# kevinh-e/BetaOne

Measured on AMD Instinct MI355X. Metric: mcts_nodes_per_sec, higher is better.
Workload: dtype f32 (3 x f16 split, f32 accumulate)

## Files before the change

### betaone_amd/csrc/bo_analyse.h

```cpp
#pragma once
#include "bo_tree.h"

#define BO_PV_CAP 16
#define BO_ANALYSIS_WORDS 32
#define ST_BAD_RANGE 128

BO_DEV bo_mv move_between(const DPos &P, const DPos &C) {
    const int us = pos_turn(P) ? BB_WHITE : BB_BLACK;
    uint64_t left = P.bb[us] & ~C.bb[us], arrived = C.bb[us] & ~P.bb[us];
    if (left & P.bb[BB_K]) { left &= P.bb[BB_K]; arrived &= C.bb[BB_K]; }
    if (!left || !arrived) return 0;
    const int from = bo_lsb64(left), to = bo_lsb64(arrived);
    int promo = 0;
    if ((P.bb[BB_P] & BIT(from)) && !(C.bb[BB_P] & BIT(to))) promo = piece_type_at(C, to);
    return MV(from, to, promo);
}

struct SetupDevArgs {
    const int *slots;
    const DPos *pos;
    long long capacity;
    const long long *first;
    const int *ply;
};
// ... 8 lines not shown
    int st = 0;
    if (ply < 0 || f < 0 || f + (long long)ply >= a.capacity) st = ST_BAD_RANGE;
    else if (ply + 1 > e.c.PLY_CAP) st = ST_PLY_OVERFLOW;
    else if (ply + 1 > e.c.TRK_CAP) st = ST_TRK_OVERFLOW;
    if (lane == 0) {
        e.status[g] = st;
        e.ctx_mode[g] = 0;
        e.stat_evals[g] = e.stat_flushes[g] = e.stat_term_sims[g] = e.stat_levels[g] = e.stat_children_scanned[g] = 0;
        e.resign_cnt[2 * g] = e.resign_cnt[2 * g + 1] = 0;
    }
    if (st) {
        if (lane == 0) {
            const size_t no = NOFF(e, g);
            e.ply[g] = 0; e.trk_n[g] = 0; e.n_hist[g] = 0;
            e.n_nodes[g] = 1; e.n_children[no] = 0; e.n_visits[no] = 0; e.q[no] = 0.0f;
            e.sims_done[g] = 0; e.rows[g] = 0; e.n_runs[g] = 0; e.n_ul[g] = 0; e.req_node[g] = -1; e.phase[g] = PH_IDLE; e.root_nch[g] = 0;
            e.root_nlegal[g] = 0; e.req_nlegal[g] = 0; e.root_term[g] = -1;
        }
        return;
    }
    DPos *gp = e.gpos + (size_t)g * e.c.PLY_CAP;
    DPos *tk = e.trk + (size_t)g * e.c.TRK_CAP;
    int *tc = e.trk_cnt + (size_t)g * e.c.TRK_CAP;
    bo_mv *pl = e.played + (size_t)g * e.c.PLY_CAP;
    for (int k0 = 0; k0 <= ply; k0 += 64) {
        const int k = k0 + lane;
        if (k <= ply) {
            DPos p = a.pos[f + k];
            if (k == 0) { p.flags |= F_IRREV; finish_key(p); }
            gp[k] = p;
            tk[k] = p;
// ... 77 lines not shown
```

### betaone_amd/csrc/bo_engine.cpp

```cpp
#include "../../include/betaone_engine.h"
#include "../../include/betaone_lab.h"

#include "bo_tree.h"
#include "bo_fastw.h"
#include "bo_select_wide.h"
#include "bo_replay.h"
#include "bo_train.h"
#include "bo_metrics.h"
#include "bo_pgn.h"
#include "bo_san.h"
#include "bo_analyse.h"
#include "bo_perft.h"
#include "bo_tb.h"
#include "bo_nn_fused.h"
#include "bo_conv.h"
#include "bo_tower.h"
#include "bo_tower_wg.h"
#include "bo_tower_h.h"
#include "bo_tower_s.h"
#include "bo_tower_s16.h"
#include "bo_tower_h16.h"
#include "bo_heads.h"
#include "bo_tower_b1.h"
#include "bo_rt.h"
// ... 205 lines not shown
    for (int k = 1; k <= cfg->mcts_batch_size; k++) {
        const double r = (double)(int)(cfg->widen_coeff * sqrt((double)k)) / (double)k;
        if (r > per_sim) per_sim = r;
    }
    c.NCAP = fast ? 2 : (int)ceil(c.S * per_sim) + 2 * root_m + 4;
    c.nstride = c.NCAP;
    c.PLY_CAP = cfg->max_plies; c.TRK_CAP = cfg->max_plies;
    c.UL_MAX = fast ? 1 : c.B; c.CH_MAX = ch_max < 1 ? 1 : ch_max;
    c.cpuct = (float)cfg->cpuct;
    c.keep = (float)(1.0 - cfg->dirichlet_epsilon);
    c.eps = cfg->dirichlet_epsilon;
    c.use_noise = cfg->dirichlet_alpha > 0 ? 1 : 0;
    c.root_m = root_m;
    c.profile = 0;
    { const char *v = getenv("BETAONE_BURST_TWO_PATHS"); c.burst_two = (v && v[0] == '0') ? 0 : 1; }
    c.root_q = 0;
    const size_t G = (size_t)c.G, N = G * (size_t)c.NCAP;
    Eng &d = e->d;
    int rc = 0;
    float *sq = nullptr, *rcp = nullptr; int *wl = nullptr;
    rc |= e->alloc(&sq, (size_t)c.S + 2); rc |= e->alloc(&wl, (size_t)c.B + 1); rc |= e->alloc(&rcp, (size_t)c.S + 3);
    int **iscal[] = {&d.sims_done, &d.n_nodes, &d.rows, &d.n_runs, &d.n_ul, &d.req_nlegal, &d.status,
                     &d.trk_n, &d.n_hist, &d.ctx_mode, &d.root_nch, &d.stat_evals,
                     &d.stat_flushes, &d.stat_term_sims, &d.stat_levels, &d.stat_children_scanned, &e->d_go, &e->d_action};
    for (int **p : iscal) rc |= e->alloc(p, G);
    const size_t res_ints = G * (4 + 2 * (size_t)BO_RES_CAP) + 4, info_ints = G * 18;
    rc |= e->alloc(&e->d_res_blk, res_ints); rc |= e->alloc(&e->d_info_blk, info_ints);
    if (!rc) {
        d.res_n = e->d_res_blk; d.res_best_idx = e->d_res_blk + G; d.res_best_mv = e->d_res_blk + 2 * G; d.res_total = e->d_res_blk + 3 * G;
        d.res_idx = e->d_res_blk + 4 * G; d.res_val = reinterpret_cast<float *>(e->d_res_blk + 4 * G + G * BO_RES_CAP);
// ... 8 lines not shown
    rc |= rt_host_alloc((void **)&e->h_res, res_ints * 4); rc |= rt_host_alloc((void **)&e->h_info, info_ints * 4);
    rc |= rt_host_alloc((void **)&e->h_noise, G * BO_MAX_MOVES * sizeof(double)); rc |= rt_host_alloc((void **)&e->h_go, G * 4);
    rc |= rt_host_alloc((void **)&e->h_action, 2 * G * 4);
    rc |= rt_host_alloc((void **)&e->h_turn_u, G * sizeof(double)); rc |= rt_host_alloc((void **)&e->h_turn_flags, G * 4);
    rc |= e->alloc(&e->d_turn_pw, (size_t)cfg->num_simulations + 1);
    { const char *v = getenv("BETAONE_TURN_COPIES"); e->ship = !(v && v[0] == '1'); }
    rc |= e->alloc(&d.gpos, G * c.PLY_CAP); rc |= e->alloc(&d.trk, G * c.TRK_CAP); rc |= e->alloc(&d.trk_cnt, G * c.TRK_CAP);
    rc |= e->alloc(&d.hist, G * 7);
    rc |= e->alloc(&d.n_visits, N); rc |= e->alloc(&d.parent, N); rc |= e->alloc(&d.first_child, N); rc |= e->alloc(&d.n_children, N);
    rc |= e->alloc(&d.q, N); rc |= e->alloc(&d.prior, N); rc |= e->alloc(&d.move, N); rc |= e->alloc(&d.term, N);
    rc |= e->alloc(&d.eval_slot, N); rc |= e->alloc(&d.npos, N);
    rc |= e->alloc(&d.run_leaf, G * c.B); rc |= e->alloc(&d.run_cnt, G * c.B);
    rc |= e->alloc(&d.ul_node, G * c.UL_MAX); rc |= e->alloc(&d.ul_nlegal, G * c.UL_MAX); rc |= e->alloc(&d.ul_value, G * c.UL_MAX);
    rc |= e->alloc(&d.ul_move, G * c.UL_MAX * BO_CH_CAP); rc |= e->alloc(&d.ul_prior, G * c.UL_MAX * BO_CH_CAP);
    rc |= e->alloc(&d.req_moves, G * BO_MAX_MOVES); rc |= e->alloc(&d.root_moves, G * BO_MAX_MOVES);
    rc |= e->alloc(&d.root_child_rank, G * 2 * BO_CH_CAP); rc |= e->alloc(&d.noise, G * BO_MAX_MOVES);
    rc |= e->alloc(&d.played, G * c.PLY_CAP);
    rc |= e->alloc(&d.prof, G * BO_PROF_SLOTS);
    rc |= e->alloc(&d.resign_cnt, 2 * G); rc |= e->alloc(&e->d_root_value, G);
    if (!rc) rt_memset(d.resign_cnt, 0, 2 * G * 4, nullptr);
    d.played_now = nullptr;
    if (fast) {
        FastW &f = e->f;
        const size_t L = (size_t)cfg->leaves_per_step;
        f.L = (int)L;
        f.sel_ut = 2; f.sel_flags = FW_SEL_OCT;
        const size_t expansions = (size_t)c.S + L + 2;
        f.NG = cfg->fast_arena_granules > 0 ? cfg->fast_arena_granules : (int)((6 * expansions + 8) * (32 / BO_FW_GR));
        if (f.NG < 64 || f.NG > BO_FW_LINK_MASK) { bo_engine_destroy(e); return fail(BO_E_ARG, "fast_arena_granules out of range (64 .. 2^24 - 1)"); }
        const size_t NR = (size_t)f.NG * BO_FW_GR;
// ... 251 lines not shown
            if (e->sel_pending) {
                float ms = 0.0f;
                RT((int)hipEventSynchronize(e->sel_ev1));
                RT((int)hipEventElapsedTime(&ms, e->sel_ev0, e->sel_ev1));
                e->sel_ms += ms; e->sel_launches++; e->sel_pending = 0;
            }
            RT((int)hipEventRecord(e->sel_ev0, (hipStream_t)stream));
        }
#endif
        RT(launch_fw_select(e, value_dev, policy_kind, stream));
#if !defined(BO_WAVE_EMU)
        if (e->sel_profile) { RT((int)hipEventRecord(e->sel_ev1, (hipStream_t)stream)); e->sel_pending = 1; }
#endif
        RT(RT_LAUNCH(bo_k_fw_leaf, rows, stream, e->d, e->f, nn_in_dev));
    } else {
        RT(RT_LAUNCH(bo_k_step, e->d.c.G, stream, e->d, policy_dev, value_dev, policy_kind, nn_in_dev, vt));
    }
    return BO_OK;
}
extern "C" int bo_step(bo_engine *e, const float *policy_dev, const float *value_dev, int policy_kind, float *nn_in_dev,
                       void *stream) {
    if (!e || !nn_in_dev) return fail(BO_E_ARG, "null argument");
    if (policy_kind != BO_POLICY_NONE && (!policy_dev || !value_dev)) return fail(BO_E_ARG, "policy/value required");
    return step_launch(e, policy_dev, value_dev, policy_kind, nn_in_dev, stream, StepTail{nullptr, nullptr, nullptr, nullptr, 0});
}
extern "C" int bo_step_heads(bo_engine *e, const float *logits_dev, const float *vpart_dev, const float *b1_dev, const float *w2_dev,
                             const float *b2_dev, int rows, float *nn_in_dev, void *stream) {
    if (!e || !nn_in_dev || !logits_dev || !vpart_dev || !b1_dev || !w2_dev || !b2_dev) return fail(BO_E_ARG, "null argument");
    if (e->fast) return fail(BO_E_CONFIG, "bo_step_heads: the reference-semantics search only (fast mode evaluates rows, not games)");
    if (rows < e->d.c.G) return fail(BO_E_ARG, "bo_step_heads: the partial sums must hold a row per game (rows >= G)");
    return step_launch(e, logits_dev, nullptr, BO_POLICY_LOGITS, nn_in_dev, stream, StepTail{vpart_dev, b1_dev, w2_dev, b2_dev, rows});
// ... 1257 lines not shown
    RT(rt_sync(stream));
    return BO_OK;
}

extern "C" int bo_debug_profile(bo_engine *e, int enable, uint64_t *cycles_out, void *stream) {
    if (!e) return fail(BO_E_ARG, "null engine");
    const size_t G = (size_t)e->d.c.G;
    if (cycles_out) {
        RT(rt_d2h(cycles_out, e->d.prof, G * BO_PROF_SLOTS * sizeof(uint64_t), stream));
        RT(rt_sync(stream));
    }
    if (enable >= 0) {
        if (enable && !e->d.c.profile) RT(rt_memset(e->d.prof, 0, G * BO_PROF_SLOTS * sizeof(uint64_t), stream));
        e->d.c.profile = enable;
    }
    return BO_OK;
}

extern "C" int bo_movegen_batch(bo_engine *e, int n, const bo_position *pos, int32_t *moves_out, int32_t *n_out,
                                int32_t *check_out, void *stream) {
    if (!e || n < 1 || !pos || !moves_out || !n_out) return fail(BO_E_ARG, "bad arguments");
    std::vector<DPos> hp((size_t)n);
    for (int i = 0; i < n; i++) hp[i] = from_abi(pos[i]);
    void *dp = nullptr, *dm = nullptr, *dn = nullptr, *dc = nullptr;
    int rc = rt_malloc(&dp, hp.size() * sizeof(DPos)) | rt_malloc(&dm, (size_t)n * BO_MAX_MOVES * sizeof(bo_mv)) |
             rt_malloc(&dn, (size_t)n * 4) | rt_malloc(&dc, (size_t)n * 4);
    std::vector<bo_mv> hm((size_t)n * BO_MAX_MOVES);
    std::vector<int> hc((size_t)n);
    if (!rc) rc = rt_h2d(dp, hp.data(), hp.size() * sizeof(DPos), stream);
    if (!rc) rc = RT_LAUNCH(bo_k_movegen, n, stream, (const DPos *)dp, (bo_mv *)dm, (int *)dn, (int *)dc);
// ... 1192 lines not shown
```

### betaone_amd/csrc/bo_tree.h

```cpp
#pragma once
#include "bo_chess.h"
#include <math.h>

#define BO_CH_CAP 32
#define BO_PATH_CAP 1024
#define BO_RES_CAP 256
#define BO_PLANES 120
#ifndef BO_PROF_SLOTS
#define BO_PROF_SLOTS 16
#endif
#define BO_ROW (BO_PLANES * 64)

enum { PH_IDLE = 0, PH_RUN = 1, PH_DONE = 2 };
enum { ST_OK = 0, ST_NODE_OVERFLOW = 1, ST_DEPTH_OVERFLOW = 2, ST_NAN_SCORE = 4, ST_PLY_OVERFLOW = 8,
       ST_ILLEGAL_ACTION = 16, ST_UL_OVERFLOW = 32, ST_TRK_OVERFLOW = 64 };
enum { POLICY_NONE = 0, POLICY_LOGITS = 1, POLICY_PROBS = 2 };

struct EngCfg {
    int G, S, B;
    int NCAP, PLY_CAP, TRK_CAP;
    int nstride;
    int UL_MAX, CH_MAX;
    float cpuct, keep;
    double eps;
    int use_noise;
    int root_m;
    int profile;
    int burst_two;
    int root_q;
};

struct Eng {
    EngCfg c;
    const float *sqrt_lut;
    const float *rcp_lut;
    const int *widen_lut;
    int *phase, *sims_done, *n_nodes, *rows, *n_runs, *n_ul, *req_node, *req_nlegal, *status;
    int *ply, *trk_n, *n_hist, *ctx_mode, *root_nlegal, *root_term, *root_nch;
    int *stat_evals, *stat_flushes, *stat_term_sims, *stat_levels, *stat_children_scanned;
    DPos *gpos, *trk, *hist;
    int *trk_cnt;
    int *n_visits, *parent, *first_child, *n_children;
    float *q, *prior;
    bo_mv *move;
    signed char *term;
    short *eval_slot;
    DPos *npos;
    int *run_leaf, *run_cnt;
    int *ul_node, *ul_nlegal;
    float *ul_value;
    bo_mv *ul_move;
    float *ul_prior;
    bo_mv *req_moves, *root_moves;
    int *root_child_rank;
    double *noise;
    bo_mv *played;
    int *res_n, *res_idx, *res_best_idx, *res_best_mv, *res_total;
    float *res_val;
    int watch_n;
    int *watch, *res_watch;
    int *played_now;
    int *resign_cnt;
    unsigned long long *prof;
};

#define NOFF(e, g) ((size_t)(g) * (size_t)(e).c.nstride)

BO_DEV float bo_expf(float x) {
// ... 196 lines not shown
BO_DEV void encode_static(const Eng &e, int g, float *row) {
    const int s = bo_lane();
    const int nh = e.n_hist[g];
    const DPos *h = e.hist + (size_t)g * 7;
    for (int pl = 0; pl < (7 - nh) * 14; pl++) row[pl * 64 + s] = 0.0f;
    for (int i = 0; i < nh; i++) {
        DPos H = h[i];
        encode_block(row, 7 - nh + i, H, tracker_reps(e, g, H));
    }
}
BO_DEV void encode_leaf(const Eng &e, int g, float *row, const DPos &P) {
    encode_block(row, 7, P, tracker_reps(e, g, P));
    encode_scalars(row, P);
}

BO_DEV int select_leaf(const Eng &e, int g, int *flags, int *path, int *depth_out, const float *lut) {
    const size_t no = NOFF(e, g);
    const int lane = bo_lane();
    int cur = 0, levels = 0, scanned = 0;
    if (lane == 0) path[0] = 0;
    int nc = e.n_children[no], fc = e.first_child[no];
    int pv = e.n_visits[no], pv_next = pv;
    for (;;) {
        if (nc == 0) break;
        const float sp = lut[pv];
        float score = -__builtin_inff();
        int n = 0, c_fc = 0, c_nc = 0;
        if (lane < nc) {
            n = e.n_visits[no + fc + lane];
            c_fc = e.first_child[no + fc + lane];
            c_nc = e.n_children[no + fc + lane];
// ... 28 lines not shown
        score = __builtin_bit_cast(float, bo_readlane(__builtin_bit_cast(int, score), 0));
        bi = bo_readlane(bi, 0);
        if (!(score > -__builtin_inff())) { *flags |= ST_NAN_SCORE; bi = 0; }
        cur = fc + bi;
        levels++;
        if (lane == 0) path[levels] = cur;
        scanned += nc;
        pv = pv_next;
        pv_next = bo_readlane(n, bi);
        fc = bo_readlane(c_fc, bi);
        nc = bo_readlane(c_nc, bi);
        if (levels >= BO_PATH_CAP - 1) { *flags |= ST_DEPTH_OVERFLOW; break; }
    }
    if (lane == 0) { e.stat_levels[g] += levels; e.stat_children_scanned[g] += scanned; }
    *depth_out = levels;
    bo_sync();
    return cur;
}

#define BO_BURST_LEVELS 4
#define BO_BURST_FITS(S) (2 * (S) + 5 <= BO_NUM_ACTIONS)
BO_DEV_NOINLINE float bo_div_general(float x, float fn) { return x / fn; }
BO_DEV float bo_div_count(float x, float fn, float y) {
    const float q0 = x * y;
    const float r = __builtin_fmaf(-fn, q0, x);
    float q = __builtin_fmaf(r, y, q0);
    const float a = q0 < 0.0f ? -q0 : q0;
    if (x == 0.0f) q = q0;
    else if (!(a >= 1e-30f && a <= 1e30f)) q = bo_div_general(x, fn);
    return q;
// ... 391 lines not shown
    BO_UNROLL
    for (int w = 0; w < 4; w++) {
        float h = 0.0f;
        BO_UNROLL
        for (int ks = 0; ks < 16; ks++) h += r.part[w][ks];
        h += r.b1[w];
        s[w] = (h > 0.0f ? h : 0.0f) * r.w2[w];
    }
    for (int m = 32; m >= 1; m >>= 1) {
        BO_UNROLL
        for (int w = 0; w < 4; w++) s[w] = s[w] + bo_shfl_xor_f(s[w], m);
    }
    return tanhf(((s[0] + s[1]) + (s[2] + s[3])) + r.b2);
}

BO_DEV void apply_leaf(const Eng &e, int g, int leaf, const float *row, int kind, const float *value_of, const StepTail &vt, StepShared &sh,
                       int *n_ul_io, int *flags) {
    const size_t no = NOFF(e, g);
    const int lane = bo_lane();
    const int n = e.req_nlegal[g];
    const bo_mv *mv = e.req_moves + (size_t)g * BO_MAX_MOVES;
    int slot = *n_ul_io;
    if (slot >= e.c.UL_MAX) { *flags |= ST_UL_OVERFLOW; slot = e.c.UL_MAX - 1; }
    const size_t uo = (size_t)g * e.c.UL_MAX + slot;
    float value;
    if (kind == POLICY_PROBS) {
        value = value_of[g];
        for (int j = lane; j < n; j += 64) sh.pv[j] = row[move_to_index(mv[j])];
    } else {
        float mx, sum;
        if (vt.vpart) {
            TailRegs tr;
            tail_load(vt, g, tr);
            row_max_sum(row, &mx, &sum);
            value = tail_value(tr);
        } else {
            value = value_of[g];
            row_max_sum(row, &mx, &sum);
        }
        for (int j = lane; j < n; j += 64) sh.pv[j] = bo_exp_row(row[move_to_index(mv[j])] - mx) / sum;
    }
    bo_sync();
    const int M = n < e.c.CH_MAX ? n : e.c.CH_MAX;
    for (int j = lane; j < n; j += 64) {
        int r = stable_rank(sh.pv, n, j);
        if (r < M) { e.ul_move[uo * BO_CH_CAP + r] = mv[j]; e.ul_prior[uo * BO_CH_CAP + r] = sh.pv[j]; }
    }
    if (lane == 0) {
        e.ul_node[uo] = leaf;
        e.ul_nlegal[uo] = n;
        e.ul_value[uo] = value;
        e.eval_slot[no + leaf] = (short)slot;
    }
    *n_ul_io = slot + 1;
    bo_sync();
}


BO_DEV int step_body(const Eng &e, int g, const float *policy, const float *value, int kind, float *nn_in, StepShared &sh, const StepTail &vt) {
    const int lane = bo_lane();
    const size_t no = NOFF(e, g);
    int flags = 0;
    int sims = e.sims_done[g], rows = e.rows[g], n_runs = e.n_runs[g], n_ul = e.n_ul[g], n_nodes = e.n_nodes[g];
    int req = e.req_node[g];
    int *rl = e.run_leaf + (size_t)g * e.c.B, *rc = e.run_cnt + (size_t)g * e.c.B;
    float *row = nn_in + (size_t)g * BO_ROW;

    const bool prof = e.c.profile != 0;
    unsigned long long pc[8] = {0, 0, 0, 0, 0, 0, 0, 0};
    int n_iter = 0, n_first = 0, n_burst = 0, n_burst_sims = 0, n_general = 0, n_swaps = 0;
    unsigned long long tk = prof ? bo_clock() : 0ull;
    const unsigned long long t_start = tk;
#define BO_PROF(slot)                                                    \
    if (prof) { const unsigned long long _n = bo_clock(); pc[slot] += _n - tk; tk = _n; }
    if (req >= 0 && kind == POLICY_NONE) return n_nodes;
    const float *lut = e.sqrt_lut;
    if (req >= 0) {
        if (req == 0) apply_root(e, g, policy + (size_t)g * BO_NUM_ACTIONS, kind, sh, &n_nodes, &flags);
        else apply_leaf(e, g, req, policy + (size_t)g * BO_NUM_ACTIONS, kind, value, vt, sh, &n_ul, &flags);
        req = -1;
    }
    BO_PROF(0)
    int phase = PH_RUN;
    bool burst_tables_staged = false;
    int term_budget = e.c.B;
    int b_depth = 0;
    float b_tv = 0.0f;
    int path_leaf = -1, path_depth = -1;
    for (;;) {
        if (sims >= e.c.S) {
            if (rows > 0) { flush_pending(e, g, n_runs, n_ul, &n_nodes, sh.path2, &flags, path_leaf, sh.path, path_depth); rows = n_runs = n_ul = 0; }
            BO_PROF(5)
            phase = PH_DONE;
            break;
        }
        int depth;
        const int leaf = select_leaf(e, g, &flags, sh.path, &depth, lut);
        path_leaf = leaf; path_depth = depth;
        n_iter++;
        BO_PROF(1)
        int t = e.term[no + leaf];
        if (t < 0) {
            n_first++;
            const DPos P = e.npos[no + leaf];
            bool chk;
            const int n = bo_movegen(P, sh.moves, &chk);
            t = terminal_eval(e, g, sh.path, depth, P, sh.moves, n, chk, sh.moves2, sh.chain);
            if (lane == 0) e.term[no + leaf] = (signed char)t;
            if (t == 0) {
                for (int j = lane; j < n; j += 64) e.req_moves[(size_t)g * BO_MAX_MOVES + j] = sh.moves[j];
                if (lane == 0) e.req_nlegal[g] = n;
            }
            bo_sync();
            BO_PROF(2)
        }
        if (t > 0) {
            const float tv = t == 1 ? 1.0f : 0.0f;
            int applied = 1;
            bool small = depth <= BO_BURST_LEVELS && BO_BURST_FITS(e.c.S);
            for (int k = 0; k < depth && small; k++) small = e.n_children[no + sh.path[k]] <= 16;
            BO_PROF(6)
            const int may = e.c.S - sims < term_budget ? e.c.S - sims : term_budget;
            if (small) {
                const bool small_b = b_depth > 0 && e.c.burst_two != 0;
                applied = terminal_burst(e, g, sh.path, depth, tv, may, sh.probs, &burst_tables_staged, sh.bpath, small_b ? b_depth : 0, b_tv, &n_swaps);
                n_burst++; n_burst_sims += applied;
                bo_sync();
                if (lane <= depth) sh.bpath[lane] = sh.path[lane];
                b_depth = depth; b_tv = tv;
                bo_sync();
            }
            else { backup_run(e, g, leaf, tv, 1, sh.path2, &flags, sh.path, depth); n_general++; }
            BO_PROF(7)
            sims += applied;
            term_budget -= applied;
            if (lane == 0) e.stat_term_sims[g] += applied;
            BO_PROF(3)
            if (term_budget <= 0 && sims < e.c.S) break;
            continue;
        }
        if (e.eval_slot[no + leaf] < 0) {
            encode_leaf(e, g, row, e.npos[no + leaf]);
            req = leaf;
            if (lane == 0) e.stat_evals[g] += 1;
            BO_PROF(4)
            break;
        }
        int cnt = e.c.B - rows;
        if (cnt > e.c.S - sims) cnt = e.c.S - sims;
        if (lane == 0) { rl[n_runs] = leaf; rc[n_runs] = cnt; }
        n_runs++;
        rows += cnt;
        sims += cnt;
        bo_sync();
        if (rows >= e.c.B) { flush_pending(e, g, n_runs, n_ul, &n_nodes, sh.path2, &flags, path_leaf, sh.path, path_depth); rows = n_runs = n_ul = 0; }
        BO_PROF(5)
    }
#undef BO_PROF
    if (prof && lane == 0) {
        const unsigned long long total = bo_clock() - t_start;
        if (e.c.profile == 1 || total > (unsigned long long)e.c.profile) {
            unsigned long long *pp = e.prof + (size_t)g * BO_PROF_SLOTS;
            pp[10] += (unsigned long long)n_burst; pp[11] += (unsigned long long)n_burst_sims; pp[12] += (unsigned long long)n_general;
            pp[13] += pc[6]; pp[14] += pc[7]; pp[15] += (unsigned long long)n_swaps;
            for (int i = 0; i < 6; i++) pp[i] += pc[i];
            pp[6] += total;
            pp[7] += 1;
            pp[8] += (unsigned long long)n_iter;
            pp[9] += (unsigned long long)n_first;
        }
    }
    if (lane == 0) {
        e.sims_done[g] = sims; e.rows[g] = rows; e.n_runs[g] = n_runs; e.n_ul[g] = n_ul; e.n_nodes[g] = n_nodes;
        e.req_node[g] = req; e.phase[g] = phase;
        if (flags) e.status[g] |= flags;
    }
    return n_nodes;
}
BO_KERNEL void bo_k_step(Eng e, const float *policy, const float *value, int kind, float *nn_in, StepTail vt) {
    BO_SHARED StepShared sh;
    const int g = bo_block();
    if (e.phase[g] != PH_RUN) return;
    step_body(e, g, policy, value, kind, nn_in, sh, vt);
}

BO_DEV int root_prepare(const Eng &e, int g, StepShared &sh) {
    const size_t no = NOFF(e, g);
    const int lane = bo_lane();
    const int ply = e.ply[g];
    const DPos P = e.gpos[(size_t)g * e.c.PLY_CAP + ply];
    if (lane == 0) {
        init_node(e, no, 0, -1, 1.0f, 0, P);
        e.n_nodes[g] = 1; e.sims_done[g] = 0; e.rows[g] = 0; e.n_runs[g] = 0; e.n_ul[g] = 0;
        e.req_node[g] = -1; e.phase[g] = PH_IDLE; e.root_nch[g] = 0;
        if (e.ctx_mode[g] == 0) {
            int nh = ply < 7 ? ply : 7;
            e.n_hist[g] = nh;
            for (int i = 0; i < nh; i++) e.hist[(size_t)g * 7 + i] = e.gpos[(size_t)g * e.c.PLY_CAP + ply - nh + i];
        }
    }
    bo_sync();
    bool chk;
    const int n = bo_movegen(P, sh.moves, &chk);
    if (lane == 0) sh.path[0] = 0;
    bo_sync();
    const int t = terminal_eval(e, g, sh.path, 0, P, sh.moves, n, chk, sh.moves2, sh.chain);
    for (int j = lane; j < n; j += 64) {
        e.root_moves[(size_t)g * BO_MAX_MOVES + j] = sh.moves[j];
        e.req_moves[(size_t)g * BO_MAX_MOVES + j] = sh.moves[j];
// ... 73 lines not shown
    const int g = bo_block();
    if (!want[g] || e.root_term[g] != 0) return;
    encode_static(e, g, nn_in + (size_t)g * BO_ROW);
    if (bo_lane() == 0) e.phase[g] = PH_RUN;
}

BO_KERNEL void bo_k_stop(Eng e, const int *mask) {
    BO_SHARED int path[BO_PATH_CAP];
    const int g = bo_block(), lane = bo_lane();
    if ((mask && !mask[g]) || e.phase[g] != PH_RUN) return;
    int flags = 0, n_nodes = e.n_nodes[g];
    if (e.rows[g] > 0) flush_pending(e, g, e.n_runs[g], e.n_ul[g], &n_nodes, path, &flags);
    bo_sync();
    if (lane == 0) {
        e.rows[g] = 0; e.n_runs[g] = 0; e.n_ul[g] = 0; e.n_nodes[g] = n_nodes;
        e.req_node[g] = -1; e.phase[g] = PH_DONE;
        if (flags) e.status[g] |= flags;
    }
}

BO_KERNEL void bo_k_ship(int *dst_a, const int *src_a, int n_a, int *dst_b, const int *src_b, int n_b, int n_blocks) {
    const int i0 = bo_block() * 64 + bo_lane(), stride = n_blocks * 64;
    for (int i = i0; i < n_a; i += stride) dst_a[i] = src_a[i];
    for (int i = i0; i < n_b; i += stride) dst_b[i] = src_b[i];
}

BO_DEV void result_body(const Eng &e, int g) {
    const int lane = bo_lane();
    if (g == 0 && lane == 0) e.res_watch[0] = e.watch ? (e.watch[0] | (e.watch_n > 1 && e.watch[1] ? 0x10000 : 0)) : 0;
    if (e.phase[g] != PH_DONE) return;
    const size_t no = NOFF(e, g);
// ... 216 lines not shown
```

### betaone_amd/csrc/bo_wave.h

```cpp
#pragma once
#include <stdint.h>

#if defined(BO_WAVE_EMU)
#include "wave_emu.h"
#else
#include <hip/hip_runtime.h>
#define BO_DEV __device__ __forceinline__
#define BO_DEV_NOINLINE __device__ __noinline__
#define BO_KERNEL extern "C" __global__ __launch_bounds__(64)
#define BO_SHARED __shared__
#define BO_CONST_TABLE __device__ const

BO_DEV int bo_lane() { return (int)(threadIdx.x & 63u); }
BO_DEV int bo_block() { return (int)blockIdx.x; }
BO_DEV uint64_t bo_ballot(bool p) { return __ballot(p); }
BO_DEV void bo_sync() { __syncthreads(); }
BO_DEV int bo_shfl(int v, int src) { return __shfl(v, src, 64); }
BO_DEV int bo_shfl_xor(int v, int m) { return __shfl_xor(v, m, 64); }
BO_DEV int bo_shfl_up(int v, int d) { return __shfl_up(v, d, 64); }
BO_DEV int bo_atomic_add(int *p, int v) { return atomicAdd(p, v); }
BO_DEV int bo_atomic_or(int *p, int v) { return atomicOr(p, v); }
BO_DEV uint64_t bo_bitrev64(uint64_t x) { return __builtin_bitreverse64(x); }
BO_DEV unsigned long long bo_clock() { return (unsigned long long)clock64(); }
#define BO_ROW_XCHG(v, kind) \
// ... 73 lines not shown
```

### betaone_amd/engine.py

```python
from __future__ import annotations

import ctypes as C
import os
from typing import Dict, List, Optional, Sequence, Tuple

import numpy as np
import torch

NUM_ACTIONS = 4672
INPUT_CHANNELS = 120
ROW_FLOATS = 120 * 64
MAX_LEGAL = 256
RES_CAP = 256
POLICY_NONE, POLICY_LOGITS, POLICY_PROBS = 0, 1, 2

STATUS_BITS = {1: "node overflow", 2: "depth overflow", 4: "NaN PUCT score", 8: "ply overflow",
               16: "illegal action", 32: "leaf cache overflow", 64: "tracker overflow", 128: "position range outside the array"}
ST_PLY_OVERFLOW, ST_ILLEGAL_ACTION = 8, 16
ST_NODE_OVERFLOW = 1


LAZY_BEGIN = "lazy-begin"


# ... 158 lines not shown
                                  C.POINTER(C.c_int64)]),
    "bo_perft": (C.c_int, [C.c_int, C.c_int32, C.POINTER(C.c_char_p), C.c_int32, C.c_int64, C.c_uint32, C.c_void_p, C.c_void_p, C.c_void_p,
                           C.POINTER(C.c_int64), C.c_void_p]),
    "bo_tb_create": (C.c_int, [C.c_int, C.c_char_p, C.POINTER(C.c_void_p), C.c_int32, C.POINTER(C.c_void_p)]),
    "bo_tb_build": (C.c_int, [C.c_void_p, C.c_int32, _I32P, C.c_void_p]),
    "bo_tb_verify": (C.c_int, [C.c_void_p, C.POINTER(C.c_uint64), C.c_void_p]),
    "bo_tb_stats": (C.c_int, [C.c_void_p, C.c_void_p]),
    "bo_tb_download": (C.c_int, [C.c_void_p, C.c_void_p, C.c_int64]),
    "bo_tb_upload": (C.c_int, [C.c_void_p, C.c_void_p, C.c_int64, C.c_int32]),
    "bo_tb_probe": (C.c_int, [C.POINTER(C.c_void_p), C.c_int32, C.c_void_p, C.c_int32, C.c_void_p, C.c_void_p, C.c_void_p]),
    "bo_tb_destroy": (None, [C.c_void_p]),
}
_LAB_SYMBOLS = {
    "bo_debug_tree": (C.c_int, [C.c_void_p, C.c_int, C.POINTER(BoNode), C.c_int32, _I32P, C.c_void_p]),
    "bo_debug_fast": (C.c_int, [C.c_void_p, C.c_int, _I32P, C.c_int32, _I32P, C.c_void_p]),
    "bo_event_pair_overhead": (C.c_int, [_F64P, C.c_int32, C.c_void_p]),
    "bo_nn_b1_profile": (C.c_int, [C.c_void_p, C.c_int, C.POINTER(C.c_uint64), C.c_int]),
    "bo_fast_stats": (C.c_int, [C.c_void_p, C.POINTER(C.c_uint64), C.POINTER(C.c_uint64), _I32P, C.c_int32, _F64P, C.POINTER(C.c_int64),
                               C.c_void_p]),
    "bo_debug_profile": (C.c_int, [C.c_void_p, C.c_int, C.POINTER(C.c_uint64), C.c_void_p]),
    "bo_debug_stamp": (C.c_int, [C.c_void_p, C.c_uint64, C.c_uint64, C.c_void_p]),
    "bo_nn_tower_forward_timed": (C.c_int, [C.c_void_p, C.c_void_p, C.c_void_p, C.c_void_p, C.c_void_p, C.c_int, C.c_void_p, C.c_void_p]),
    "bo_select_wide": (C.c_int, [C.c_void_p, C.c_void_p, C.c_void_p, C.c_void_p, C.c_int, C.c_int, C.c_float, C.c_int,
                                 C.c_void_p, C.c_void_p, C.c_void_p]),
}

HIP_LIB_PATH = os.path.join(os.path.dirname(os.path.abspath(__file__)), "csrc", "libbetaone_hip.so")


def bind(cdll: C.CDLL) -> C.CDLL:
# ... 344 lines not shown
        self._check(self.lib.bo_debug_tree(self.h, slot, arr, n.value, C.byref(n), stream))
        return [dict(parent=a.parent, n=a.n_visits, q=np.float32(a.q_value), prior=np.float32(a.prior), move=a.move,
                     n_children=a.n_children, first_child=a.first_child, terminal=a.terminal) for a in arr[:n.value]]

    def status(self, stream: int = 0) -> Dict[str, np.ndarray]:
        names = ["status", "evals", "flushes", "term_sims", "levels", "children_scanned"]
        out = {k: np.zeros(self.G, np.int32) for k in names}
        self._check(self.lib.bo_engine_status(self.h, *[_p(out[k]) for k in names], stream))
        return out

    def fast_options(self, tree_reuse=None, games_per_halfwave=None, select_flags=None):
        self._check(self.lib.bo_fast_options(self.h, -1 if tree_reuse is None else (1 if tree_reuse else 0),
                                             -1 if games_per_halfwave is None else int(games_per_halfwave),
                                             -1 if select_flags is None else int(select_flags)))

    SEL_NT, SEL_ROOT_IN_REGS, SEL_DENSE, SEL_LANE, SEL_OCT, SEL_QUAD = 1, 2, 4, 8, 16, 32
    def debug_fast(self, slot: int, stream: int = 0):
        L = self.L
        cs = (16 + 7 * L + 31) // 32 * 32
        ctl, paths = np.zeros(cs, np.int32), np.zeros((L, 64), np.int32)
        self._check(self.lib.bo_debug_fast(self.h, slot, _p(ctl), cs, _p(paths), stream))
        names = ["row_slot", "row_plink", "row_nlegal", "row_term", "row_sim", "sim_row", "sim_plen"]
        out = dict(n_rows=int(ctl[0]), n_step=int(ctl[1]), cur=int(ctl[2]), top=int(ctl[3]), levels=int(ctl[4]), kids=int(ctl[5]),
                   granules=int(ctl[6]), path_nodes=int(ctl[7]), term_sims=int(ctl[8]))
        for i, nm in enumerate(names):
            out[nm] = ctl[16 + i * L:16 + (i + 1) * L].copy()
        return out, paths

    GRANULE_BYTES = 128

# ... 54 lines not shown
```

### include/betaone_lab.h

```cpp
#ifndef BETAONE_LAB_H
#define BETAONE_LAB_H

#include "betaone_engine.h"

#ifdef __cplusplus
extern "C" {
#endif

#define BO_PROF_SLOTS 16

typedef struct {
    int32_t parent, n_visits, first_child, n_children;
    float q_value, prior;
    int32_t move;
    int32_t terminal;
} bo_node;
int bo_debug_tree(bo_engine *e, int slot, bo_node *out, int32_t cap, int32_t *n_nodes, void *stream);

int bo_fast_stats(bo_engine *e, uint64_t *granules_read, uint64_t *path_nodes, int32_t *arena_granules, int32_t time_select, double *select_ms,
                  int64_t *select_launches, void *stream);

int bo_event_pair_overhead(double *ms_out, int32_t samples, void *stream);

int bo_debug_fast(bo_engine *e, int slot, int32_t *ctl_out, int32_t ctl_cap, int32_t *paths_out, void *stream);

int bo_debug_profile(bo_engine *e, int enable, uint64_t *cycles_out, void *stream);

int bo_select_wide(const void *blocks_dev, const int32_t *root_block_dev, const int32_t *root_n_dev,
                   const float *sqrt_lut_dev, int n_trees, int max_depth, float cpuct, int grid_blocks,
                   int32_t *out_leaf_dev, int32_t *out_levels_dev, void *stream);

int bo_nn_tower_forward_timed(bo_tower *tower, const float *x_dev, float *y_dev, void *head_a_dev, void *head_b_dev, int batch,
// ... 11 lines not shown
```

Before: 74.18 million.

## Resume step from saved leaf path instead of re-descending after NN eval

Each game now saves the selected leaf's path, depth and scan count when it issues an NN request. The next step kernel applies the leaf and continues from that saved path instead of running select_leaf again from the root. The step kernel is also templated on tail and profiling flags so the unused branches compile out, and per-game head state is loaded up front and pinned in registers. The cost is extra memory for the path plus one extra store per request, and the resumed path skips the term check, which relies on the leaf's state not having changed in between.

```diff
diff --git a/betaone_amd/csrc/bo_analyse.h b/betaone_amd/csrc/bo_analyse.h
--- a/betaone_amd/csrc/bo_analyse.h
+++ b/betaone_amd/csrc/bo_analyse.h
@@ -46,7 +46,7 @@
             const size_t no = NOFF(e, g);
             e.ply[g] = 0; e.trk_n[g] = 0; e.n_hist[g] = 0;
             e.n_nodes[g] = 1; e.n_children[no] = 0; e.n_visits[no] = 0; e.q[no] = 0.0f;
-            e.sims_done[g] = 0; e.rows[g] = 0; e.n_runs[g] = 0; e.n_ul[g] = 0; e.req_node[g] = -1; e.phase[g] = PH_IDLE; e.root_nch[g] = 0;
+            e.sims_done[g] = 0; e.rows[g] = 0; e.n_runs[g] = 0; e.n_ul[g] = 0; e.req_node[g] = -1; e.req_depth[g] = -1; e.phase[g] = PH_IDLE; e.root_nch[g] = 0;
             e.root_nlegal[g] = 0; e.req_nlegal[g] = 0; e.root_term[g] = -1;
         }
         return;
diff --git a/betaone_amd/csrc/bo_engine.cpp b/betaone_amd/csrc/bo_engine.cpp
--- a/betaone_amd/csrc/bo_engine.cpp
+++ b/betaone_amd/csrc/bo_engine.cpp
@@ -243,6 +243,7 @@
     c.root_m = root_m;
     c.profile = 0;
     { const char *v = getenv("BETAONE_BURST_TWO_PATHS"); c.burst_two = (v && v[0] == '0') ? 0 : 1; }
+    { const char *v = getenv("BETAONE_STEP_REDESCEND"); c.redescend = (v && v[0] == '1') ? 1 : 0; }
     c.root_q = 0;
     const size_t G = (size_t)c.G, N = G * (size_t)c.NCAP;
     Eng &d = e->d;
@@ -281,6 +282,11 @@
     rc |= e->alloc(&d.ul_node, G * c.UL_MAX); rc |= e->alloc(&d.ul_nlegal, G * c.UL_MAX); rc |= e->alloc(&d.ul_value, G * c.UL_MAX);
     rc |= e->alloc(&d.ul_move, G * c.UL_MAX * BO_CH_CAP); rc |= e->alloc(&d.ul_prior, G * c.UL_MAX * BO_CH_CAP);
     rc |= e->alloc(&d.req_moves, G * BO_MAX_MOVES); rc |= e->alloc(&d.root_moves, G * BO_MAX_MOVES);
+    rc |= e->alloc(&d.req_path, G * BO_PATH_CAP); rc |= e->alloc(&d.req_depth, G); rc |= e->alloc(&d.req_scanned, G);
+    if (!rc) {
+        rt_memset(d.req_path, 0, G * BO_PATH_CAP * sizeof(int), nullptr); rt_memset(d.req_depth, 0xFF, G * sizeof(int), nullptr);
+        rt_memset(d.req_scanned, 0, G * sizeof(int), nullptr); rt_memset(d.req_moves, 0, G * BO_MAX_MOVES * sizeof(bo_mv), nullptr);
+    }
     rc |= e->alloc(&d.root_child_rank, G * 2 * BO_CH_CAP); rc |= e->alloc(&d.noise, G * BO_MAX_MOVES);
     rc |= e->alloc(&d.played, G * c.PLY_CAP);
     rc |= e->alloc(&d.prof, G * BO_PROF_SLOTS);
@@ -562,7 +568,15 @@
 #endif
         RT(RT_LAUNCH(bo_k_fw_leaf, rows, stream, e->d, e->f, nn_in_dev));
     } else {
-        RT(RT_LAUNCH(bo_k_step, e->d.c.G, stream, e->d, policy_dev, value_dev, policy_kind, nn_in_dev, vt));
+#if defined(BO_WAVE_EMU)
+        RT(RT_LAUNCH((bo_k_step<true, true>), e->d.c.G, stream, e->d, policy_dev, value_dev, policy_kind, nn_in_dev, vt));
+#else
+        const bool tail = vt.vpart != nullptr, prof = e->d.c.profile != 0;
+        if (tail && prof) RT(RT_LAUNCH((bo_k_step<true, true>), e->d.c.G, stream, e->d, policy_dev, value_dev, policy_kind, nn_in_dev, vt));
+        else if (tail) RT(RT_LAUNCH((bo_k_step<true, false>), e->d.c.G, stream, e->d, policy_dev, value_dev, policy_kind, nn_in_dev, vt));
+        else if (prof) RT(RT_LAUNCH((bo_k_step<false, true>), e->d.c.G, stream, e->d, policy_dev, value_dev, policy_kind, nn_in_dev, NoTail{}));
+        else RT(RT_LAUNCH((bo_k_step<false, false>), e->d.c.G, stream, e->d, policy_dev, value_dev, policy_kind, nn_in_dev, NoTail{}));
+#endif
     }
     return BO_OK;
 }
@@ -1850,6 +1864,16 @@
         if (enable && !e->d.c.profile) RT(rt_memset(e->d.prof, 0, G * BO_PROF_SLOTS * sizeof(uint64_t), stream));
         e->d.c.profile = enable;
     }
+    return BO_OK;
+}
+
+extern "C" int bo_debug_req_path(bo_engine *e, int slot, int32_t *depth_out, int32_t *scanned_out, int32_t *path_out, int32_t cap, void *stream) {
+    if (!e || slot < 0 || slot >= e->d.c.G || !depth_out) return fail(BO_E_ARG, "bad arguments");
+    if (cap > BO_PATH_CAP) cap = BO_PATH_CAP;
+    RT(rt_d2h(depth_out, e->d.req_depth + slot, 4, stream));
+    if (scanned_out) RT(rt_d2h(scanned_out, e->d.req_scanned + slot, 4, stream));
+    if (path_out && cap > 0) RT(rt_d2h(path_out, e->d.req_path + (size_t)slot * BO_PATH_CAP, (size_t)cap * 4, stream));
+    RT(rt_sync(stream));
     return BO_OK;
 }
 
diff --git a/betaone_amd/csrc/bo_tree.h b/betaone_amd/csrc/bo_tree.h
--- a/betaone_amd/csrc/bo_tree.h
+++ b/betaone_amd/csrc/bo_tree.h
@@ -28,6 +28,7 @@
     int profile;
     int burst_two;
     int root_q;
+    int redescend;
 };
 
 struct Eng {
@@ -52,6 +53,8 @@
     bo_mv *ul_move;
     float *ul_prior;
     bo_mv *req_moves, *root_moves;
+    int *req_path;
+    int *req_depth, *req_scanned;
     int *root_child_rank;
     double *noise;
     bo_mv *played;
@@ -278,7 +281,7 @@
     encode_scalars(row, P);
 }
 
-BO_DEV int select_leaf(const Eng &e, int g, int *flags, int *path, int *depth_out, const float *lut) {
+BO_DEV int select_leaf(const Eng &e, int g, int *flags, int *path, int *depth_out, const float *lut, int *scanned_out = nullptr) {
     const size_t no = NOFF(e, g);
     const int lane = bo_lane();
     int cur = 0, levels = 0, scanned = 0;
@@ -337,6 +340,7 @@
     }
     if (lane == 0) { e.stat_levels[g] += levels; e.stat_children_scanned[g] += scanned; }
     *depth_out = levels;
+    if (scanned_out) *scanned_out = scanned;
     bo_sync();
     return cur;
 }
@@ -758,11 +762,12 @@
     return tanhf(((s[0] + s[1]) + (s[2] + s[3])) + r.b2);
 }
 
-BO_DEV void apply_leaf(const Eng &e, int g, int leaf, const float *row, int kind, const float *value_of, const StepTail &vt, StepShared &sh,
-                       int *n_ul_io, int *flags) {
+struct NoTail {};
+template <bool TAIL, class Tail>
+BO_DEV void apply_leaf(const Eng &e, int g, int leaf, const float *row, int kind, const float *value_of, const Tail &vt, StepShared &sh,
+                       int n, bo_mv mv0, int *n_ul_io, int *flags) {
     const size_t no = NOFF(e, g);
     const int lane = bo_lane();
-    const int n = e.req_nlegal[g];
     const bo_mv *mv = e.req_moves + (size_t)g * BO_MAX_MOVES;
     int slot = *n_ul_io;
     if (slot >= e.c.UL_MAX) { *flags |= ST_UL_OVERFLOW; slot = e.c.UL_MAX - 1; }
@@ -770,25 +775,30 @@
     float value;
     if (kind == POLICY_PROBS) {
         value = value_of[g];
-        for (int j = lane; j < n; j += 64) sh.pv[j] = row[move_to_index(mv[j])];
+        for (int j = lane; j < n; j += 64) sh.pv[j] = row[move_to_index(j < 64 ? mv0 : mv[j])];
     } else {
         float mx, sum;
-        if (vt.vpart) {
-            TailRegs tr;
-            tail_load(vt, g, tr);
-            row_max_sum(row, &mx, &sum);
-            value = tail_value(tr);
-        } else {
+        bool tail = false;
+        if constexpr (TAIL) tail = vt.vpart != nullptr;
+        if constexpr (TAIL) {
+            if (tail) {
+                TailRegs tr;
+                tail_load(vt, g, tr);
+                row_max_sum(row, &mx, &sum);
+                value = tail_value(tr);
+            }
+        }
+        if (!tail) {
             value = value_of[g];
             row_max_sum(row, &mx, &sum);
         }
-        for (int j = lane; j < n; j += 64) sh.pv[j] = bo_exp_row(row[move_to_index(mv[j])] - mx) / sum;
+        for (int j = lane; j < n; j += 64) sh.pv[j] = bo_exp_row(row[move_to_index(j < 64 ? mv0 : mv[j])] - mx) / sum;
     }
     bo_sync();
     const int M = n < e.c.CH_MAX ? n : e.c.CH_MAX;
     for (int j = lane; j < n; j += 64) {
         int r = stable_rank(sh.pv, n, j);
-        if (r < M) { e.ul_move[uo * BO_CH_CAP + r] = mv[j]; e.ul_prior[uo * BO_CH_CAP + r] = sh.pv[j]; }
+        if (r < M) { e.ul_move[uo * BO_CH_CAP + r] = j < 64 ? mv0 : mv[j]; e.ul_prior[uo * BO_CH_CAP + r] = sh.pv[j]; }
     }
     if (lane == 0) {
         e.ul_node[uo] = leaf;
@@ -801,30 +811,109 @@
 }
 
 
-BO_DEV int step_body(const Eng &e, int g, const float *policy, const float *value, int kind, float *nn_in, StepShared &sh, const StepTail &vt) {
+struct StepHead {
+    int phase, sims, rows, n_runs, n_ul, n_nodes, req, nlegal, depth, scanned;
+    int path0;
+    bo_mv mv0;
+};
+BO_DEV void step_head_load(const Eng &e, int g, StepHead &h) {
+    const int lane = bo_lane();
+    h.sims = e.sims_done[g]; h.rows = e.rows[g]; h.n_runs = e.n_runs[g]; h.n_ul = e.n_ul[g]; h.n_nodes = e.n_nodes[g];
+    h.req = e.req_node[g]; h.nlegal = e.req_nlegal[g]; h.depth = e.req_depth[g]; h.scanned = e.req_scanned[g];
+    h.path0 = e.req_path[(size_t)g * BO_PATH_CAP + lane];
+    h.mv0 = e.req_moves[(size_t)g * BO_MAX_MOVES + lane];
+    h.phase = e.phase[g];
+}
+BO_DEV void step_head_pin(const StepHead &h) {
+#if !defined(BO_WAVE_EMU)
+    asm volatile("" ::"s"(h.phase), "s"(h.sims), "s"(h.rows), "s"(h.n_runs), "s"(h.n_ul), "s"(h.n_nodes), "s"(h.req), "s"(h.nlegal), "s"(h.depth),
+                 "s"(h.scanned), "v"(h.path0), "v"((int)h.mv0));
+#else
+    (void)h;
+#endif
+}
+
+#if defined(BO_WAVE_EMU)
+#define BO_DEV_M inline
+#else
+#define BO_DEV_M __device__ __forceinline__
+#endif
+template <bool PROF> struct StepProf {
+    bool on;
+    unsigned long long pc[8], tk, t_start;
+    int n_iter, n_first, n_burst, n_burst_sims, n_general, n_swaps;
+    BO_DEV_M void start(const Eng &e) {
+        on = e.c.profile != 0;
+        for (int i = 0; i < 8; i++) pc[i] = 0;
+        n_iter = n_first = n_burst = n_burst_sims = n_general = n_swaps = 0;
+        tk = on ? bo_clock() : 0ull;
+        t_start = tk;
+    }
+    BO_DEV_M void phase(int slot) {
+        if (on) { const unsigned long long n = bo_clock(); pc[slot] += n - tk; tk = n; }
+    }
+    BO_DEV_M void iter() { n_iter++; }
+    BO_DEV_M void first() { n_first++; }
+    BO_DEV_M void burst(int applied) { n_burst++; n_burst_sims += applied; }
+    BO_DEV_M void general() { n_general++; }
+    BO_DEV_M int *swaps() { return &n_swaps; }
+    BO_DEV_M void finish(const Eng &e, int g) {
+        if (on && bo_lane() == 0) {
+            const unsigned long long total = bo_clock() - t_start;
+            if (e.c.profile == 1 || total > (unsigned long long)e.c.profile) {
+                unsigned long long *pp = e.prof + (size_t)g * BO_PROF_SLOTS;
+                pp[10] += (unsigned long long)n_burst; pp[11] += (unsigned long long)n_burst_sims; pp[12] += (unsigned long long)n_general;
+                pp[13] += pc[6]; pp[14] += pc[7]; pp[15] += (unsigned long long)n_swaps;
+                for (int i = 0; i < 6; i++) pp[i] += pc[i];
+                pp[6] += total;
+                pp[7] += 1;
+                pp[8] += (unsigned long long)n_iter;
+                pp[9] += (unsigned long long)n_first;
+            }
+        }
+    }
+};
+template <> struct StepProf<false> {
+    BO_DEV_M void start(const Eng &) {}
+    BO_DEV_M void phase(int) {}
+    BO_DEV_M void iter() {}
+    BO_DEV_M void first() {}
+    BO_DEV_M void burst(int) {}
+    BO_DEV_M void general() {}
+    BO_DEV_M int *swaps() { return nullptr; }
+    BO_DEV_M void finish(const Eng &, int) {}
+};
+
+template <bool TAIL, bool PROF, class Tail>
+BO_DEV int step_body(const Eng &e, int g, const StepHead &h, const float *policy, const float *value, int kind, float *nn_in, StepShared &sh,
+                     const Tail &vt) {
     const int lane = bo_lane();
     const size_t no = NOFF(e, g);
     int flags = 0;
-    int sims = e.sims_done[g], rows = e.rows[g], n_runs = e.n_runs[g], n_ul = e.n_ul[g], n_nodes = e.n_nodes[g];
-    int req = e.req_node[g];
+    int sims = h.sims, rows = h.rows, n_runs = h.n_runs, n_ul = h.n_ul, n_nodes = h.n_nodes;
+    int req = h.req;
     int *rl = e.run_leaf + (size_t)g * e.c.B, *rc = e.run_cnt + (size_t)g * e.c.B;
     float *row = nn_in + (size_t)g * BO_ROW;
 
-    const bool prof = e.c.profile != 0;
-    unsigned long long pc[8] = {0, 0, 0, 0, 0, 0, 0, 0};
-    int n_iter = 0, n_first = 0, n_burst = 0, n_burst_sims = 0, n_general = 0, n_swaps = 0;
-    unsigned long long tk = prof ? bo_clock() : 0ull;
-    const unsigned long long t_start = tk;
-#define BO_PROF(slot)                                                    \
-    if (prof) { const unsigned long long _n = bo_clock(); pc[slot] += _n - tk; tk = _n; }
+    StepProf<PROF> pf;
+    pf.start(e);
     if (req >= 0 && kind == POLICY_NONE) return n_nodes;
     const float *lut = e.sqrt_lut;
+    int resume_leaf = -1, resume_depth = -1;
     if (req >= 0) {
         if (req == 0) apply_root(e, g, policy + (size_t)g * BO_NUM_ACTIONS, kind, sh, &n_nodes, &flags);
-        else apply_leaf(e, g, req, policy + (size_t)g * BO_NUM_ACTIONS, kind, value, vt, sh, &n_ul, &flags);
+        else {
+            apply_leaf<TAIL>(e, g, req, policy + (size_t)g * BO_NUM_ACTIONS, kind, value, vt, sh, h.nlegal, h.mv0, &n_ul, &flags);
+            if (h.depth >= 0 && e.c.redescend == 0) {
+                if (lane <= h.depth) sh.path[lane] = h.path0;
+                for (int i = lane + 64; i <= h.depth; i += 64) sh.path[i] = e.req_path[(size_t)g * BO_PATH_CAP + i];
+                bo_sync();
+                resume_leaf = req; resume_depth = h.depth;
+            }
+        }
         req = -1;
     }
-    BO_PROF(0)
+    pf.phase(0);
     int phase = PH_RUN;
     bool burst_tables_staged = false;
     int term_budget = e.c.B;
@@ -834,18 +923,23 @@
     for (;;) {
         if (sims >= e.c.S) {
             if (rows > 0) { flush_pending(e, g, n_runs, n_ul, &n_nodes, sh.path2, &flags, path_leaf, sh.path, path_depth); rows = n_runs = n_ul = 0; }
-            BO_PROF(5)
+            pf.phase(5);
             phase = PH_DONE;
             break;
         }
-        int depth;
-        const int leaf = select_leaf(e, g, &flags, sh.path, &depth, lut);
+        int depth, scanned = 0, leaf;
+        const bool resumed = resume_leaf >= 0;
+        if (resumed) {
+            leaf = resume_leaf; depth = resume_depth;
+            resume_leaf = -1;
+            if (lane == 0) { e.stat_levels[g] += depth; e.stat_children_scanned[g] += h.scanned; }
+        } else leaf = select_leaf(e, g, &flags, sh.path, &depth, lut, &scanned);
         path_leaf = leaf; path_depth = depth;
-        n_iter++;
-        BO_PROF(1)
-        int t = e.term[no + leaf];
+        pf.iter();
+        pf.phase(1);
+        int t = resumed ? 0 : (int)e.term[no + leaf];
         if (t < 0) {
-            n_first++;
+            pf.first();
             const DPos P = e.npos[no + leaf];
             bool chk;
             const int n = bo_movegen(P, sh.moves, &chk);
@@ -856,38 +950,42 @@
                 if (lane == 0) e.req_nlegal[g] = n;
             }
             bo_sync();
-            BO_PROF(2)
+            pf.phase(2);
         }
         if (t > 0) {
             const float tv = t == 1 ? 1.0f : 0.0f;
             int applied = 1;
             bool small = depth <= BO_BURST_LEVELS && BO_BURST_FITS(e.c.S);
             for (int k = 0; k < depth && small; k++) small = e.n_children[no + sh.path[k]] <= 16;
-            BO_PROF(6)
+            pf.phase(6);
             const int may = e.c.S - sims < term_budget ? e.c.S - sims : term_budget;
             if (small) {
                 const bool small_b = b_depth > 0 && e.c.burst_two != 0;
-                applied = terminal_burst(e, g, sh.path, depth, tv, may, sh.probs, &burst_tables_staged, sh.bpath, small_b ? b_depth : 0, b_tv, &n_swaps);
-                n_burst++; n_burst_sims += applied;
+                applied = terminal_burst(e, g, sh.path, depth, tv, may, sh.probs, &burst_tables_staged, sh.bpath, small_b ? b_depth : 0, b_tv, pf.swaps());
+                pf.burst(applied);
                 bo_sync();
                 if (lane <= depth) sh.bpath[lane] = sh.path[lane];
                 b_depth = depth; b_tv = tv;
                 bo_sync();
             }
-            else { backup_run(e, g, leaf, tv, 1, sh.path2, &flags, sh.path, depth); n_general++; }
-            BO_PROF(7)
+            else { backup_run(e, g, leaf, tv, 1, sh.path2, &flags, sh.path, depth); pf.general(); }
+            pf.phase(7);
             sims += applied;
             term_budget -= applied;
             if (lane == 0) e.stat_term_sims[g] += applied;
-            BO_PROF(3)
+            pf.phase(3);
             if (term_budget <= 0 && sims < e.c.S) break;
             continue;
         }
-        if (e.eval_slot[no + leaf] < 0) {
+        if (!resumed && e.eval_slot[no + leaf] < 0) {
             encode_leaf(e, g, row, e.npos[no + leaf]);
             req = leaf;
+            if (e.c.redescend == 0) {
+                for (int i = lane; i <= depth; i += 64) e.req_path[(size_t)g * BO_PATH_CAP + i] = sh.path[i];
+                if (lane == 0) { e.req_depth[g] = depth; e.req_scanned[g] = scanned; }
+            }
             if (lane == 0) e.stat_evals[g] += 1;
-            BO_PROF(4)
+            pf.phase(4);
             break;
         }
         int cnt = e.c.B - rows;
@@ -898,22 +996,9 @@
         sims += cnt;
         bo_sync();
         if (rows >= e.c.B) { flush_pending(e, g, n_runs, n_ul, &n_nodes, sh.path2, &flags, path_leaf, sh.path, path_depth); rows = n_runs = n_ul = 0; }
-        BO_PROF(5)
-    }
-#undef BO_PROF
-    if (prof && lane == 0) {
-        const unsigned long long total = bo_clock() - t_start;
-        if (e.c.profile == 1 || total > (unsigned long long)e.c.profile) {
-            unsigned long long *pp = e.prof + (size_t)g * BO_PROF_SLOTS;
-            pp[10] += (unsigned long long)n_burst; pp[11] += (unsigned long long)n_burst_sims; pp[12] += (unsigned long long)n_general;
-            pp[13] += pc[6]; pp[14] += pc[7]; pp[15] += (unsigned long long)n_swaps;
-            for (int i = 0; i < 6; i++) pp[i] += pc[i];
-            pp[6] += total;
-            pp[7] += 1;
-            pp[8] += (unsigned long long)n_iter;
-            pp[9] += (unsigned long long)n_first;
-        }
-    }
+        pf.phase(5);
+    }
+    pf.finish(e, g);
     if (lane == 0) {
         e.sims_done[g] = sims; e.rows[g] = rows; e.n_runs[g] = n_runs; e.n_ul[g] = n_ul; e.n_nodes[g] = n_nodes;
         e.req_node[g] = req; e.phase[g] = phase;
@@ -921,11 +1006,17 @@
     }
     return n_nodes;
 }
-BO_KERNEL void bo_k_step(Eng e, const float *policy, const float *value, int kind, float *nn_in, StepTail vt) {
+template <bool TAIL> struct StepTailArg { typedef StepTail type; };
+template <> struct StepTailArg<false> { typedef NoTail type; };
+template <bool TAIL, bool PROF>
+BO_KERNEL_T void bo_k_step(Eng e, const float *policy, const float *value, int kind, float *nn_in, typename StepTailArg<TAIL>::type vt) {
     BO_SHARED StepShared sh;
     const int g = bo_block();
-    if (e.phase[g] != PH_RUN) return;
-    step_body(e, g, policy, value, kind, nn_in, sh, vt);
+    StepHead h;
+    step_head_load(e, g, h);
+    step_head_pin(h);
+    if (h.phase != PH_RUN) return;
+    step_body<TAIL, PROF>(e, g, h, policy, value, kind, nn_in, sh, vt);
 }
 
 BO_DEV int root_prepare(const Eng &e, int g, StepShared &sh) {
@@ -936,7 +1027,7 @@
     if (lane == 0) {
         init_node(e, no, 0, -1, 1.0f, 0, P);
         e.n_nodes[g] = 1; e.sims_done[g] = 0; e.rows[g] = 0; e.n_runs[g] = 0; e.n_ul[g] = 0;
-        e.req_node[g] = -1; e.phase[g] = PH_IDLE; e.root_nch[g] = 0;
+        e.req_node[g] = -1; e.req_depth[g] = -1; e.phase[g] = PH_IDLE; e.root_nch[g] = 0;
         if (e.ctx_mode[g] == 0) {
             int nh = ply < 7 ? ply : 7;
             e.n_hist[g] = nh;
@@ -1040,7 +1131,7 @@
     bo_sync();
     if (lane == 0) {
         e.rows[g] = 0; e.n_runs[g] = 0; e.n_ul[g] = 0; e.n_nodes[g] = n_nodes;
-        e.req_node[g] = -1; e.phase[g] = PH_DONE;
+        e.req_node[g] = -1; e.req_depth[g] = -1; e.phase[g] = PH_DONE;
         if (flags) e.status[g] |= flags;
     }
 }
diff --git a/betaone_amd/csrc/bo_wave.h b/betaone_amd/csrc/bo_wave.h
--- a/betaone_amd/csrc/bo_wave.h
+++ b/betaone_amd/csrc/bo_wave.h
@@ -3,11 +3,13 @@
 
 #if defined(BO_WAVE_EMU)
 #include "wave_emu.h"
+#define BO_KERNEL_T static
 #else
 #include <hip/hip_runtime.h>
 #define BO_DEV __device__ __forceinline__
 #define BO_DEV_NOINLINE __device__ __noinline__
 #define BO_KERNEL extern "C" __global__ __launch_bounds__(64)
+#define BO_KERNEL_T __global__ __launch_bounds__(64)
 #define BO_SHARED __shared__
 #define BO_CONST_TABLE __device__ const
 
diff --git a/betaone_amd/engine.py b/betaone_amd/engine.py
--- a/betaone_amd/engine.py
+++ b/betaone_amd/engine.py
@@ -196,6 +196,7 @@
 _LAB_SYMBOLS = {
     "bo_debug_tree": (C.c_int, [C.c_void_p, C.c_int, C.POINTER(BoNode), C.c_int32, _I32P, C.c_void_p]),
     "bo_debug_fast": (C.c_int, [C.c_void_p, C.c_int, _I32P, C.c_int32, _I32P, C.c_void_p]),
+    "bo_debug_req_path": (C.c_int, [C.c_void_p, C.c_int, _I32P, _I32P, _I32P, C.c_int32, C.c_void_p]),
     "bo_event_pair_overhead": (C.c_int, [_F64P, C.c_int32, C.c_void_p]),
     "bo_nn_b1_profile": (C.c_int, [C.c_void_p, C.c_int, C.POINTER(C.c_uint64), C.c_int]),
     "bo_fast_stats": (C.c_int, [C.c_void_p, C.POINTER(C.c_uint64), C.POINTER(C.c_uint64), _I32P, C.c_int32, _F64P, C.POINTER(C.c_int64),
@@ -570,6 +571,11 @@
                                              -1 if games_per_halfwave is None else int(games_per_halfwave),
                                              -1 if select_flags is None else int(select_flags)))
 
+    def req_path(self, slot: int, stream: int = 0):
+        depth, scanned, path = C.c_int32(-1), C.c_int32(0), np.zeros(1024, np.int32)
+        self._check(self.lib.bo_debug_req_path(self.h, slot, C.byref(depth), C.byref(scanned), _p(path), len(path), stream))
+        return depth.value, scanned.value, path[:max(depth.value + 1, 0)].copy()
+
     SEL_NT, SEL_ROOT_IN_REGS, SEL_DENSE, SEL_LANE, SEL_OCT, SEL_QUAD = 1, 2, 4, 8, 16, 32
     def debug_fast(self, slot: int, stream: int = 0):
         L = self.L
diff --git a/include/betaone_lab.h b/include/betaone_lab.h
--- a/include/betaone_lab.h
+++ b/include/betaone_lab.h
@@ -16,6 +16,8 @@
     int32_t terminal;
 } bo_node;
 int bo_debug_tree(bo_engine *e, int slot, bo_node *out, int32_t cap, int32_t *n_nodes, void *stream);
+
+int bo_debug_req_path(bo_engine *e, int slot, int32_t *depth_out, int32_t *scanned_out, int32_t *path_out, int32_t cap, void *stream);
 
 int bo_fast_stats(bo_engine *e, uint64_t *granules_read, uint64_t *path_nodes, int32_t *arena_granules, int32_t time_select, double *select_ms,
                   int64_t *select_launches, void *stream);
```

Result: no change. 74.88 million, median of 6 (+0.9%).
